# dotchen/LearningByCheating

Hardware: AMD Instinct MI355X
Metric: images/sec ImagePolicyModelSS phase-1 train @ bs256 (higher is better)
Workload: dtype bf16; 1 GPU; ImagePolicyModelSS(resnet34) phase-1 step vs BirdViewPolicyModelSS(resnet18) teacher [phase1_bs256_bf16], 160x384 RGB + 7x192x192 bird-view uint8 NHWC frames as the dataset stores them (2048-frame dataset per rank resident in HBM, a different batch every step), global batch 256 (256/GPU), bf16 MFMA operands and bf16 activation storage + f32 accumulate/master weights/gradients/BN/loss/Adam, local B; global_batch=256, parallelism=dp1

## Files before the change

learningbycheating_amd/csrc/conv_hdma.hip:

```cpp
#include "lbc_common.hpp"
#include "lbc_act.hpp"
#include "conv_lds_dma.hpp"


namespace {

struct HdmaCfg { int bm, bn, hrmax; };
const HdmaCfg kHdmaCfg[kLbcHdmaCfgs] = {{0, 0, 0}, {256, 128, 384}, {128, 256, 192}, {256, 64, 456}, {128, 64, 192}};
constexpr long long kHdmaSmallMinTiles = 48;

}

int lbc_conv_hdma_pick(const IgemmArgs& a, int mode)
{
    if (lbc_opt_on(kOptNoHdma) || lbc_opt_on(kOptNoGemm256)) return -1;
    if (a.nphase == 4) {
        if (!lbc_conv_hdmap_phased(a, mode) || lbc_opt(kOptGemm256Cfg) >= 0) return -1;
        const long long forcedp = lbc_opt(kOptHdmaCfg);
        if (forcedp >= 0 && forcedp != 4) return -1;
        const long long tiles = (long long)lbc_cdiv(a.M, 128) * (a.K / 64);
        const long long small_fill = lbc_opt(kOptGemm256MinTiles) > 0 ? lbc_opt(kOptGemm256MinTiles) : kHdmaSmallMinTiles;
        return tiles >= small_fill ? kLbcCfgHdma + 4 : -1;
    }
    if (!(a.w_bf16 && a.act_bf16) || a.ostep != 1 || a.nphase > 1 || a.oy0 || a.ox0) return -1;
    const bool c64 = a.C == 64 && a.K == 64;
    if (a.pre_scale && (mode != 0 || !c64 || lbc_opt_on(kOptNoC64pPre) || a.resid != nullptr)) return -1;
    if (a.KH != 3 || a.KW != 3 || a.P != 1 || a.S != 1 || a.C % 64 || (mode != 0 && mode != 1)) return -1;
    if (a.H != a.OH || a.W != a.OW || a.M != a.N * a.H * a.W || (long long)a.N * a.H * a.W * a.C >= (1ll << 31)) return -1;
    if ((long long)a.K * 9 * a.C >= (1ll << 31)) return -1;
    const long long fill = lbc_opt(kOptGemm256MinTiles) > 0 ? lbc_opt(kOptGemm256MinTiles) : 96;
    const long long forced = lbc_opt(kOptHdmaCfg);
    if (c64) {
        if (forced >= 0 && forced != 3) return -1;
        if (256 + 2 * a.W + 2 >= kHdmaCfg[3].hrmax || lbc_cdiv(a.M, 256) < fill) return -1;
        return kLbcCfgHdma + 3;
    }
    int best = -1;
    long long best_tiles = 0;
    double best_score = 0.0;
    for (int i = 1; i < 3; ++i) {
        const HdmaCfg& c = kHdmaCfg[i];
        if (a.K % c.bn) continue;
// ... 6 lines not shown
    }
    const long long below = lbc_opt(kOptHdmaSmallBelow) >= 0 ? lbc_opt(kOptHdmaSmallBelow) : 160;
    const bool prefer_small = best >= 0 && forced < 0 && best_tiles < below && a.K % 64 == 0 && lbc_opt(kOptGemm256MinTiles) <= 0 &&
                              lbc_conv_hdmap_eligible(a, mode, kLbcCfgHdma + 4);
    if (best >= 0 && !prefer_small) return kLbcCfgHdma + best;
    if ((forced < 0 || forced == 4) && a.K % 64 == 0 && lbc_conv_hdmap_eligible(a, mode, kLbcCfgHdma + 4)) {
        const long long tiles = (long long)lbc_cdiv(a.M, 128) * (a.K / 64);
        const long long small_fill = lbc_opt(kOptGemm256MinTiles) > 0 ? lbc_opt(kOptGemm256MinTiles) : kHdmaSmallMinTiles;
        if (tiles >= small_fill) return kLbcCfgHdma + 4;
    }
    return -1;
}

int lbc_conv_hdma_rows(const IgemmArgs& a, int cfg)
{
    if (cfg == kLbcCfgHdma + 3) return lbc_conv_c64p_rows(a);
    return lbc_cdiv(a.M, kHdmaCfg[cfg - kLbcCfgHdma].bm);
}

int lbc_conv_hdma_launch(const IgemmArgs& a, int mode, int cfg, hipStream_t s)
{
    LBC_REQUIRE(cfg > kLbcCfgHdma && cfg < kLbcCfgHdma + kLbcHdmaCfgs, "conv_hdma: bad cfg %d", cfg);
    const HdmaCfg c = kHdmaCfg[cfg - kLbcCfgHdma];
    LBC_REQUIRE(a.K % c.bn == 0 && a.C % 64 == 0 && c.bm + (a.nphase == 4 ? 1 : 2) * a.W + 2 < c.hrmax, "conv_hdma: shape not tileable");
    if (cfg == kLbcCfgHdma + 3) return lbc_conv_c64p_launch(a, mode, s);
    return lbc_conv_hdmap_launch(a, mode, cfg, s);
}
```

learningbycheating_amd/csrc/conv_hdmap.hip:

```cpp
#include "lbc_common.hpp"
#include "lbc_act.hpp"
#include "conv_hdmap.hpp"

int lbc_conv_hdmap_launch_256x128_320(const IgemmArgs& a, int mode, const void* zero, int ntiles, int tpw, unsigned grid, hipStream_t s);
int lbc_conv_hdmap_launch_256x128_384(const IgemmArgs& a, int mode, const void* zero, int ntiles, int tpw, unsigned grid, hipStream_t s);
int lbc_conv_hdmap_launch_128x256_192(const IgemmArgs& a, int mode, const void* zero, int ntiles, int tpw, unsigned grid, hipStream_t s);
int lbc_conv_hdmap_launch_128x64_192(const IgemmArgs& a, int mode, const void* zero, int ntiles, int tpw, unsigned grid, hipStream_t s, int nsplit, int kgroups);

namespace {

template <bool FUSED>
__global__ __launch_bounds__(256) void conv_split_epilogue_k(IgemmArgs a, const int nsplit)
{
    __shared__ float red[2][32][64];
    const int tid = threadIdx.x, rg = tid >> 3, seg = tid & 7;
    const int mt = blockIdx.x, n0 = blockIdx.y * 64, col = n0 + seg * 8;
    const size_t plane = (size_t)a.M * (size_t)a.K;
    __bf16* y = static_cast<__bf16*>(a.y);
    const __bf16* resid = static_cast<const __bf16*>(a.resid);
    const __bf16* by = static_cast<const __bf16*>(a.bnb_y);
    const __bf16* bmask = static_cast<const __bf16*>(a.bnb_mask);
    size_t o[4];
    bool live[4];
    f32x8 v[4];
#pragma unroll
    for (int q = 0; q < 4; ++q) {
        const int m = mt * 128 + rg + 32 * q;
        live[q] = m < a.M;
        o[q] = (size_t)(live[q] ? m : 0) * (size_t)a.K + (size_t)col;
        v[q] = ParamVec<8>::ld(a.split_ws + o[q]);
// ... 33 lines not shown
            u1 += t; u2 += t * t;
        }
        if (live[q]) *reinterpret_cast<bf16x8*>(y + o[q]) = ch;
    }
    if (a.stats) {
#pragma unroll
        for (int e = 0; e < 8; ++e) { red[0][rg][seg * 8 + e] = u1[e]; red[1][rg][seg * 8 + e] = u2[e]; }
        __syncthreads();
        if (tid < 128) {
            const int which = tid >> 6, c = tid & 63;
            float sum = 0.f;
#pragma unroll
            for (int r = 0; r < 32; ++r) sum += red[which][r][c];
            a.stats[(size_t)(a.stat_row0 + mt) * 2 * (size_t)a.K + (size_t)which * (size_t)a.K + (size_t)(n0 + c)] = sum;
        }
    }
}

}

int lbc_conv_hdmap_nsplit(const IgemmArgs& a, int mode, int cfg)
{
    (void)mode;
    if (cfg != kLbcCfgHdma + 4 || !a.split_ws || a.pre_scale || a.nphase == 4) return 1;
    const long long opt = lbc_opt(kOptHdmapSplit);
    if (opt == 0) return 1;
    const int nslab = a.C / 64;
    const long long tiles = (long long)lbc_cdiv(a.M, 128) * (a.K / 64), elems = (long long)a.M * a.K;
    auto fits = [&](long long n) { return n > 1 && nslab % n == 0 && elems * n <= a.split_ws_floats && elems * n < (1ll << 31); };
    if (opt > 1) return fits(opt) ? (int)opt : 1;
    if (tiles > 64 || nslab < 8) return 1;
    return fits(4) ? 4 : 1;
}

bool lbc_conv_hdmap_phased(const IgemmArgs& a, int mode)
{
    return mode == 1 && a.nphase == 4 && a.S == 2 && a.ostep == 2 && a.KH == 3 && a.KW == 3 && a.P == 1 && a.H == a.LH && a.W == a.LW &&
           a.OH == 2 * a.LH && a.OW == 2 * a.LW && a.M == a.N * a.LH * a.LW && !a.resid && !a.bnb_y && !a.pre_scale && a.w_bf16 && a.act_bf16 &&
           a.C % 64 == 0 && a.K % 64 == 0 && 128 + a.W + 2 <= 192 - 8 && (long long)a.N * a.OH * a.OW * a.K < (1ll << 31) &&
           (long long)a.N * a.H * a.W * a.C < (1ll << 31) && (long long)a.K * 9 * a.C < (1ll << 31) && !lbc_opt_on(kOptNoGldsPhased);
}

bool lbc_conv_hdmap_eligible(const IgemmArgs& a, int mode, int cfg)
{
    if (a.nphase == 4) return cfg == kLbcCfgHdma + 4 && lbc_conv_hdmap_phased(a, mode);
    if (mode != 0 && mode != 1) return false;
    if (a.pre_scale) return false;
    if (a.bnb_y && (mode != 1 || (a.resid != nullptr) != (a.bnb_mask != nullptr))) return false;
    if (cfg == kLbcCfgHdma + 1) return 256 + 2 * a.W + 2 <= 384 - 8;
    if (cfg == kLbcCfgHdma + 2 || cfg == kLbcCfgHdma + 4) return 128 + 2 * a.W + 2 <= 192 - 8;
    return false;
}

int lbc_conv_hdmap_launch(const IgemmArgs& a, int mode, int cfg, hipStream_t s)
{
    LBC_REQUIRE(lbc_conv_hdmap_eligible(a, mode, cfg), "conv_hdmap: launch not eligible");
    const int bm = cfg == kLbcCfgHdma + 1 ? 256 : 128, bn = cfg == kLbcCfgHdma + 1 ? 128 : (cfg == kLbcCfgHdma + 4 ? 64 : 256);
    LBC_REQUIRE(a.K % bn == 0 && a.C % 64 == 0, "conv_hdmap: shape not tileable");
    const void* zero = nullptr;
    int rc = lbc_zero_page(&zero);
    if (rc) return rc;
    const int ntiles = lbc_cdiv(a.M, bm) * (a.K / bn);
    const int cap = lbc_opt(kOptHdmaPersistWgs) > 0 ? (int)lbc_opt(kOptHdmaPersistWgs) : (cfg == kLbcCfgHdma + 4 ? 512 : 256);
    if (a.nphase == 4) {
        const int tpwp = lbc_cdiv(ntiles, cap);
        return lbc_conv_hdmap_launch_128x64_192(a, 2, zero, ntiles, tpwp, (unsigned)lbc_cdiv(ntiles, tpwp), s, 1, 1);
    }
    const int nsplit = lbc_conv_hdmap_nsplit(a, mode, cfg);
    if (nsplit > 1) {
        rc = lbc_conv_hdmap_launch_128x64_192(a, mode, zero, ntiles, 1, (unsigned)(ntiles * nsplit), s, nsplit, 1);
        if (rc) return rc;
        const dim3 eg((unsigned)lbc_cdiv(a.M, 128), (unsigned)(a.K / 64));
        if (a.bnb_y) hipLaunchKernelGGL(conv_split_epilogue_k<true>, eg, dim3(256), 0, s, a, nsplit);
        else hipLaunchKernelGGL(conv_split_epilogue_k<false>, eg, dim3(256), 0, s, a, nsplit);
        return lbc_check_launch("conv_split_epilogue");
    }
    if (cfg == kLbcCfgHdma + 4 && ntiles <= 256 && (a.C / 64) % 2 == 0 && (lbc_opt(kOptHdmapSplit) < 0 || lbc_opt(kOptHdmapSplit) == 1) && lbc_opt(kOptHdmaPersistWgs) <= 0)
        return lbc_conv_hdmap_launch_128x64_192(a, mode, zero, ntiles, 1, (unsigned)ntiles, s, 1, 2);
    const int tpw = lbc_cdiv(ntiles, cap);
    const unsigned grid = (unsigned)lbc_cdiv(ntiles, tpw);
    if (cfg == kLbcCfgHdma + 1) {
        if (256 + 2 * a.W + 2 <= 320 - 8) return lbc_conv_hdmap_launch_256x128_320(a, mode, zero, ntiles, tpw, grid, s);
        return lbc_conv_hdmap_launch_256x128_384(a, mode, zero, ntiles, tpw, grid, s);
    }
    if (cfg == kLbcCfgHdma + 4) return lbc_conv_hdmap_launch_128x64_192(a, mode, zero, ntiles, tpw, grid, s, 1, 1);
    return lbc_conv_hdmap_launch_128x256_192(a, mode, zero, ntiles, tpw, grid, s);
}
```

learningbycheating_amd/csrc/conv_hdmap.hpp:

```cpp
#pragma once
#include <type_traits>
#include "lbc_common.hpp"
#include "lbc_act.hpp"
#include "conv_lds_dma.hpp"

namespace {

#define LBC_SG(mask, n) __builtin_amdgcn_sched_group_barrier((mask), (n), 0)

__device__ __forceinline__ const char* uniform_ptr(const char* p)
{
    const unsigned long long v = (unsigned long long)(size_t)p;
    const unsigned lo = __builtin_amdgcn_readfirstlane((unsigned)v), hi = __builtin_amdgcn_readfirstlane((unsigned)(v >> 32));
    return reinterpret_cast<const char*>((size_t)(((unsigned long long)hi << 32) | lo));
}

template <int BM, int BN, int WM, int WN, int HRMAX, int SROWS>
constexpr int hdmap_lds_bytes() { return 2 * HRMAX * 128 + 3 * BN * 128 + WM * WN * SROWS * ((BN / WN) * 2 + 16) + WM * 2 * BN * 4; }
template <int BM, int BN, int WM, int WN, int HRMAX, int SROWS, int MODE, int EPI, int KG = 1>
__global__ __launch_bounds__(WM * WN * 64 * KG, (BM / WM == 128 && WM * WN == 4) ? 1 : 2) void conv_hdmap_k(IgemmArgs a, const void* zero_page, const int ntiles, const int tpw, const int nsplit)
{
    static_assert(KG == 1 || (KG == 2 && WM * WN == 4 && EPI != 3), "conv_hdmap: the in-workgroup K split doubles the four-wave shape");
    static_assert(MODE != 2 || (WM * WN == 4 && EPI == 0 && KG == 1), "conv_hdmap: the phased transposed form is a plain-epilogue form of the four-wave shape");
    constexpr int NPH = MODE == 2 ? 4 : 1;
    constexpr int WTM = BM / WM, WTN = BN / WN;
    constexpr int MT = WTM / 32, NT = WTN / 32;
    constexpr int NW = WM * WN;
    static_assert((NW == 8 || NW == 4) && (NT == 2 || NT == 1) && (MT == 2 || MT == 4), "conv_hdmap: wave tiling");
    static_assert(HRMAX % (8 * NW) == 0 && BN % (8 * NW) == 0 && (SROWS == 8 || SROWS == 16), "conv_hdmap: staging");
    constexpr int NB = 3;
    constexpr int KS = 4;
    constexpr int ABYTES = HRMAX * 128;
    constexpr int TILE_B = BN * 128;
    constexpr int BRING = 2 * ABYTES;
    constexpr int SROW_B = WTN * 2 + 16;
    constexpr int STG = BRING + NB * TILE_B;
    constexpr int RED = STG + NW * SROWS * SROW_B;
    constexpr int SMEM = RED + WM * 2 * BN * 4;
    static_assert(SMEM == hdmap_lds_bytes<BM, BN, WM, WN, HRMAX, SROWS>(), "conv_hdmap: LDS layout");
    constexpr int ZROW = (HRMAX - 1) * 128;
    static_assert(SMEM * KG <= 160 * 1024, "conv_hdmap: LDS");
    __shared__ __attribute__((aligned(16))) char smem_all[SMEM * KG];
    constexpr int HPW = HRMAX / (8 * NW);
    constexpr int NBW = BN / (8 * NW);
    constexpr int ATAPS = 7;
    constexpr int PPT = (HPW + ATAPS - 1) / ATAPS;
    static_assert(PPT >= 1 && PPT <= 2, "conv_hdmap: halo pieces per tap");
    constexpr int NSTEP = WTM / SROWS;
    constexpr int SEGS = WTN / 8;
    constexpr int CPL = SROWS * SEGS / 64;
    constexpr int RPP = 64 / SEGS;
    constexpr int NST = NSTEP * CPL;

    const int lane = threadIdx.x & 63;
    const int wave_all = __builtin_amdgcn_readfirstlane((int)threadIdx.x >> 6);
    const int grp = KG == 2 ? wave_all / NW : 0;
    const int wave = KG == 2 ? wave_all % NW : wave_all;
    const int tid = wave * 64 + lane;
    char* const smem = smem_all + grp * SMEM;
    const int wm = wave / WN, wn = wave % WN;
    const int l31 = lane & 31, kh = lane >> 5;
    const int W = a.W, H = a.H, C = a.C;
    const int ntn = a.K / BN;
    const int nslab = EPI == 3 ? C / 64 / nsplit : C / 64 / KG;

    int first, cnt, split = 0;
    {
        const int nwg = gridDim.x, b = blockIdx.x;
        const int xcd = b & 7, q = nwg >> 3, rr = nwg & 7;
        const int p = (xcd < rr ? xcd * (q + 1) : rr * (q + 1) + (xcd - rr) * q) + (b >> 3);
        if constexpr (EPI == 3) {
            first = p / nsplit;
            split = p - first * nsplit;
            cnt = first < ntiles ? 1 : 0;
        } else {
            first = p * tpw;
            cnt = ntiles - first < tpw ? ntiles - first : tpw;
        }
    }
    if (cnt <= 0) return;

    const __bf16* xin = static_cast<const __bf16*>(a.x) + (EPI == 3 ? split * nslab * 64 : (KG == 2 ? grp * nslab * 64 : 0));
    const __bf16* win = static_cast<const __bf16*>(a.w) + (EPI == 3 ? split * nslab * 64 : (KG == 2 ? grp * nslab * 64 : 0));
    const int prow = lane >> 3, pseg = lane & 7;

    const int HR = MODE == 2 ? BM + W + 2 : BM + 2 * W + 2;
    const int hshift = MODE == 2 ? 0 : W + 1;
    const int arow0 = wave * HPW * 8 + prow;
    const unsigned aswz[2] = {(unsigned)((pseg ^ ((arow0 >> 1) & 7)) * 16), (unsigned)((pseg ^ (((arow0 >> 1) + 4) & 7)) * 16)};
    const unsigned zoff = (unsigned)((lane & 7) * 16);
    const char* xbytes = reinterpret_cast<const char*>(xin);
    const char* zbytes = static_cast<const char*>(zero_page);
    auto issue_a = [&](const int m0x, const int slab, const int buf, const int j) {
        const bool pad = (wave * HPW + j) * 8 >= HR;
        int q = m0x - hshift + arow0 + 8 * j;
        q = q < 0 ? 0 : (q >= a.M ? a.M - 1 : q);
        const unsigned off = (unsigned)q * (unsigned)(2 * C) + aswz[j & 1];
        const char* sbase = uniform_ptr(pad ? zbytes : xbytes + (size_t)(slab * 128));
        lds_dma16(sbase + (pad ? zoff : off), smem + buf * ABYTES + (wave * HPW + j) * 1024);
    };
    unsigned voffb[NBW];
#pragma unroll
    for (int j = 0; j < NBW; ++j) {
        const int row = (wave * NBW + j) * 8 + prow;
        voffb[j] = (unsigned)row * (unsigned)(18 * C) + (unsigned)((pseg ^ ((row >> 1) & 7)) * 16);
    }
    const char* wbytes = reinterpret_cast<const char*>(win);
    auto issue_b = [&](const int n0x, const int slab, const int tap, const int slot, const int j0, const int j1) {
        char* base = smem + BRING + slot * TILE_B;
        const char* wsrc = uniform_ptr(wbytes + ((size_t)n0x * (size_t)(18 * C) + (size_t)(2 * (tap * C + slab * 64))));
#pragma unroll
        for (int j = 0; j < NBW; ++j)
            if (j >= j0 && j < j1) lds_dma16(wsrc + voffb[j], base + (wave * NBW + j) * 1024);
    };
    const int baddr = (BRING + (wn * WTN + l31) * 128) | ((kh ^ ((l31 >> 1) & 7)) << 4);
    int rowc[MT];
#pragma unroll
    for (int i = 0; i < MT; ++i) rowc[i] = hshift + wm * WTM + i * 32 + l31;
    auto tap_mask = [&](const int m0x, int (&mask)[MT]) {
#pragma unroll
        for (int i = 0; i < MT; ++i) {
            const int m = m0x + wm * WTM + i * 32 + l31;
            int bits = 0;
            if (m < a.M) {
                const int x = m % W;
                const int y = (m / W) % H;
#pragma unroll
                for (int t = 0; t < 9; ++t) {
                    const int r = t / 3, s = t - 3 * r;
                    const int dy = MODE == 0 ? r - 1 : (MODE == 2 ? (r == 0 ? 1 : 0) : 1 - r);
                    const int dx = MODE == 0 ? s - 1 : (MODE == 2 ? (s == 0 ? 1 : 0) : 1 - s);
                    if ((unsigned)(y + dy) < (unsigned)H && (unsigned)(x + dx) < (unsigned)W) bits |= 1 << t;
                }
            }
            mask[i] = bits;
        }
    };
    int amask[MT], amaskn[MT];

    f32x16 acc[NPH][MT][NT];
    auto zero_acc = [&]() {
#pragma unroll
        for (int p = 0; p < NPH; ++p)
#pragma unroll
            for (int i = 0; i < MT; ++i)
#pragma unroll
                for (int j = 0; j < NT; ++j)
#pragma unroll
                    for (int r = 0; r < 16; ++r) acc[p][i][j][r] = 0.f;
    };
    zero_acc();

    int aaddr[MT];
    auto tap_addr = [&](const int tap, const int buf, const int (&mask)[MT]) {
        const int r = tap / 3, s = tap - 3 * r;
        const int off = MODE == 0 ? (r - 1) * W + (s - 1) : (MODE == 2 ? (r == 0 ? W : 0) + (s == 0 ? 1 : 0) : (1 - r) * W + (1 - s));
        const int abuf = buf * ABYTES;
#pragma unroll
        for (int i = 0; i < MT; ++i) {
            const int hr = rowc[i] + off;
            const int val = (hr << 7) | ((kh ^ ((hr >> 1) & 7)) << 4), zval = ZROW | (kh << 4);
            const int m = -((mask[i] >> tap) & 1);
            aaddr[i] = abuf + (((val ^ zval) & m) ^ zval);
        }
    };

    bf16x8 fa[2][MT], fb[2][NT];
    constexpr bool ASMRD = NB * TILE_B + (NT - 1) * 4096 < 65536;
    const unsigned lds0 = (unsigned)(size_t)(__attribute__((address_space(3))) char*)smem_all + (unsigned)(grp * SMEM);
#ifdef LBC_HIP_EMULATED_FOR_TESTS
#define LBC_RD1(DST, ADDR, OFF) DST = *reinterpret_cast<const bf16x8*>(smem + (ADDR) + (OFF))
#define LBC_USE(SET) do { } while (0)
#else
#define LBC_RD1(DST, ADDR, OFF)                                                                                                  \
    do {                                                                                                                         \
        if constexpr (ASMRD) asm volatile("ds_read_b128 %0, %1 offset:%2" : "=v"(DST) : "v"(lds0 + (unsigned)(ADDR)), "n"(OFF)); \
        else DST = *reinterpret_cast<const bf16x8*>(smem + (ADDR) + (OFF));                                                      \
    } while (0)
#define LBC_USE(SET)                                                                                                             \
// ... 7 lines not shown
#define LBC_WAIT_OLDER_READS() do { if constexpr (ASMRD) __builtin_amdgcn_s_waitcnt(waitcnt_imm(63, MT + NT)); } while (0)
#define LBC_RD(SLOT, G, SET)                                                                                                     \
    do {                                                                                                                         \
        _Pragma("unroll") for (int i = 0; i < MT; ++i) LBC_RD1(fa[SET][i], aaddr[i] ^ (32 * (G)), 0);                            \
        if constexpr (NT == 2) { LBC_RD1(fb[SET][0], baddr ^ (32 * (G)), (SLOT) * TILE_B); LBC_RD1(fb[SET][NT - 1], baddr ^ (32 * (G)), (SLOT) * TILE_B + 4096); } \
        else LBC_RD1(fb[SET][0], baddr ^ (32 * (G)), (SLOT) * TILE_B);                                                           \
    } while (0)
#define LBC_MM(SET, PHX)                                                                                                         \
    do {                                                                                                                         \
        _Pragma("unroll") for (int i = 0; i < MT; ++i)                                                                           \
            _Pragma("unroll") for (int j = 0; j < NT; ++j)                                                                       \
                acc[PHX][i][j] = __builtin_amdgcn_mfma_f32_32x32x16_bf16(fa[SET][i], fb[SET][j], acc[PHX][i][j], 0, 0, 0);       \
    } while (0)

    auto wait_vm = [&](const int n) {
        switch (n) {
#define LBC_WV(N) case N: LBC_WAIT_VM(N); break;
            LBC_WV(1) LBC_WV(2) LBC_WV(3) LBC_WV(4) LBC_WV(5) LBC_WV(6) LBC_WV(7) LBC_WV(8) LBC_WV(9) LBC_WV(10) LBC_WV(11) LBC_WV(12)
            LBC_WV(13) LBC_WV(14) LBC_WV(15) LBC_WV(16) LBC_WV(17) LBC_WV(18) LBC_WV(19) LBC_WV(20) LBC_WV(21) LBC_WV(22) LBC_WV(23) LBC_WV(24)
#undef LBC_WV
            default: LBC_WAIT_VM(0); break;
        }
    };
    static_assert(NBW + 2 * PPT + NPH * NST <= 24, "conv_hdmap: counted waits");

    int tile = first;
    int mtile = tile / ntn, n0 = (tile - mtile * ntn) * BN, m0 = mtile * BM;
    int sg = 0;
    tap_mask(m0, amask);

#pragma unroll
    for (int j = 0; j < HPW; ++j) issue_a(m0, 0, 0, j);
    issue_b(n0, 0, 0, 0, 0, NBW);
    issue_b(n0, 0, 1, 1, 0, NBW);
    LBC_WAIT_VM(NBW);
    __builtin_amdgcn_s_barrier();
    tap_addr(0, 0, amask);
    LBC_RD(0, 0, 0);
    bool stores_pending = false;
    for (int it = 0; it < cnt; ++it) {
        const bool more = it + 1 < cnt;
        const int tilen = tile + 1;
        const int mtilen = tilen / ntn, n0n = (tilen - mtilen * ntn) * BN, m0n = mtilen * BM;
        if (more) tap_mask(m0n, amaskn);

        auto slab_body = [&](const int c, auto last_tag) {
            constexpr bool LAST = decltype(last_tag)::value;
            const bool follows = !LAST || more;
#pragma unroll
            for (int i = 0; i < MT; ++i) asm volatile("" : "+v"(rowc[i]), "+v"(amask[i]));
            const int buf = sg & 1;
#pragma unroll
            for (int t = 0; t < 9; ++t) {
                const int slot = t % 3, nslot = (t + 1) % 3, islot = (t + 2) % 3;
                const int tph = MODE == 2 ? (t / 3 == 1 ? 0 : 2) + (t % 3 == 1 ? 0 : 1) : 0;
                const bool has_next = t < 8 || follows;
                const bool w2 = t + 2 < 9 || follows;
                const int np_here = (t * PPT < HPW ? (HPW - t * PPT < PPT ? HPW - t * PPT : PPT) : 0);
                const int np_prev = t >= 1 ? ((t - 1) * PPT < HPW ? (HPW - (t - 1) * PPT < PPT ? HPW - (t - 1) * PPT : PPT) : 0) : 0;
                const bool hp = np_here > 0 && follows;
                auto issue_w = [&](const int j0, const int j1) {
                    if (!w2) return;
                    const int tt = t + 2 < 9 ? t + 2 : t - 7;
                    const int cc = t + 2 < 9 ? c : (LAST ? 0 : c + 1);
                    const int nn = (t + 2 < 9 || !LAST) ? n0 : n0n;
                    issue_b(nn, cc, tt, islot, j0, j1);
                };
                auto issue_h = [&]() {
                    if (!hp) return;
#pragma unroll
                    for (int q = 0; q < PPT; ++q)
                        if (t * PPT + q < HPW) {
                            if (!LAST) issue_a(m0, c + 1, buf ^ 1, t * PPT + q);
                            else issue_a(m0n, 0, buf ^ 1, t * PPT + q);
                        }
                };
#pragma unroll
                for (int g = 0; g + 1 < KS; ++g) {
                    LBC_RD(slot, g + 1, (g + 1) & 1);
                    if (g == KS - 2 && has_next) {
                        if (t < 8) tap_addr(t + 1, buf, amask);
                        else if (!LAST) tap_addr(0, buf ^ 1, amask);
                        else tap_addr(0, buf ^ 1, amaskn);
                    }
                    if (g == 0) issue_w(0, NBW / 2);
                    else if (g == 1) issue_w(NBW / 2, NBW);
                    else issue_h();
                    LBC_WAIT_OLDER_READS();
                    LBC_USE(g & 1);
                    LBC_MM(g & 1, tph);
                    LBC_SG(0x100, MT + NT);
#pragma unroll
                    for (int q = 0; q < MT * NT; ++q) { LBC_SG(0x008, 1); LBC_SG(0x036, 5); }
                    __builtin_amdgcn_sched_barrier(0);
                }
                {
                    int n = 0;
                    if (w2) {
                        n = NBW + (follows ? np_prev + np_here : 0);
                        if (c == 0 && t == 0 && stores_pending) n += NPH * NST;
                    }
                    wait_vm(n);
                }
                LBC_WAIT_LGKM0();
                __builtin_amdgcn_s_barrier();
                __builtin_amdgcn_sched_barrier(0);
                if (has_next) LBC_RD(nslot, 0, 0);
                LBC_USE((KS - 1) & 1);
                LBC_MM((KS - 1) & 1, tph);
                LBC_SG(0x100, MT + NT);
#pragma unroll
                for (int q = 0; q < MT * NT; ++q) { LBC_SG(0x008, 1); LBC_SG(0x036, 6); }
                __builtin_amdgcn_sched_barrier(0);
            }
            ++sg;
        };
        for (int c = 0; c + 1 < nslab; ++c) slab_body(c, std::false_type{});
        slab_body(nslab - 1, std::true_type{});

        if constexpr (KG == 2) {
            static_assert(NW * MT * NT * 16 * 64 * 4 <= 2 * ABYTES, "conv_hdmap: accumulator hand-over buffer");
            float* xch = reinterpret_cast<float*>(smem_all + SMEM) + (size_t)wave * (MT * NT * 16 * 64) + lane;
// ... 176 lines not shown
                            red[(wm * 2 + 1) * BN + wn * WTN + nj * 32 + l31] = s2[nj];
                        }
                    }
                }
                LBC_WAIT_LGKM0();
                __builtin_amdgcn_s_barrier();
                if (epi_on && tid < BN) {
                    float u1 = 0.f, u2 = 0.f;
#pragma unroll
                    for (int w2 = 0; w2 < WM; ++w2) { u1 += red[(w2 * 2 + 0) * BN + tid]; u2 += red[(w2 * 2 + 1) * BN + tid]; }
                    float* dst = a.stats + (size_t)(a.stat_row0 + ph * (ntiles / ntn) + mtile) * 2 * (size_t)a.K;
                    dst[n0 + tid] = u1;
                    dst[a.K + n0 + tid] = u2;
                }
                if constexpr (NPH > 1) { LBC_WAIT_LGKM0(); __builtin_amdgcn_s_barrier(); }
            }
            }
        }
        zero_acc();
        stores_pending = true;
        tile = tilen; mtile = mtilen; n0 = n0n; m0 = m0n;
#pragma unroll
        for (int i = 0; i < MT; ++i) amask[i] = amaskn[i];
    }
#undef LBC_RD
#undef LBC_RD1
#undef LBC_USE
#undef LBC_WAIT_OLDER_READS
#undef LBC_MM
}
#undef LBC_SG

template <int BM, int BN, int WM, int WN, int HRMAX, int SROWS>
int conv_hdmap_launch_shape(const IgemmArgs& a, int mode, const void* zero, int ntiles, int tpw, dim3 grid, hipStream_t s, int nsplit = 1, int kgroups = 1)
{
    if (nsplit > 1) {
        if constexpr (BM == 128 && BN == 64) {
            LBC_REQUIRE(a.split_ws && tpw == 1 && grid.x == (unsigned)(ntiles * nsplit) && (a.C / 64) % nsplit == 0, "conv_hdmap: bad split-K launch");
            if (mode == 0) hipLaunchKernelGGL((conv_hdmap_k<BM, BN, WM, WN, HRMAX, SROWS, 0, 3>), grid, dim3(WM * WN * 64), 0, s, a, zero, ntiles, tpw, nsplit);
            else hipLaunchKernelGGL((conv_hdmap_k<BM, BN, WM, WN, HRMAX, SROWS, 1, 3>), grid, dim3(WM * WN * 64), 0, s, a, zero, ntiles, tpw, nsplit);
            return lbc_check_launch("conv_hdmap(split)");
        } else {
            LBC_REQUIRE(false, "conv_hdmap: split-K exists for the 128 x 64 shape only");
        }
    }
    const int epi = a.bnb_y ? (a.bnb_mask ? 4 : 2) : (a.resid ? 1 : 0);
// ... 41 lines not shown
```

learningbycheating_amd/csrc/conv_igemm.hip:

```cpp
#include "lbc_common.hpp"
#include "lbc_act.hpp"
#include <type_traits>
#include <stdlib.h>

namespace {

template <int BM, int BN, bool WMAJOR, int MODE, bool BF16, typename AT, typename WT, int PF, int BKV = 0, bool X3 = false>
__global__ __launch_bounds__(256, PF == 2 ? 2 : 1) void conv_igemm_k(IgemmArgs a)
{
    static_assert(!BF16 || WMAJOR, "the bf16 path needs depth-contiguous weights");
    static_assert(!X3 || (BF16 && !Act<AT>::kBf16 && !Act<WT>::kBf16), "the split path reads f32 tensors and f32 weights");
    static_assert(!Act<AT>::kBf16 || BF16, "bf16 activations need the bf16 MFMA path");
    static_assert(!Act<WT>::kBf16 || BF16, "bf16 weights need the bf16 MFMA path");
    constexpr bool ABF = Act<AT>::kBf16;
    constexpr bool WBF = Act<WT>::kBf16;
    using breg_t = typename std::conditional<WBF, bf16x8, f32x4>::type;
    constexpr int BEL = WBF ? 8 : 4;
    using areg_t = typename std::conditional<ABF, bf16x8, f32x4>::type;
    using lds_t = typename std::conditional<BF16, __bf16, float>::type;
    constexpr int BK = BKV ? BKV : (BF16 ? 64 : 32);
    constexpr int LDK = (X3 ? 2 * BK : BK) + (BF16 ? 8 : 4);
    constexpr int LO = X3 ? BK : 0;
    constexpr int SEGS = BK / BEL;
    constexpr int RPP = 256 / SEGS;
// ... 498 lines not shown
    LBC_REQUIRE(!a.bf16 || wmajor, "igemm: the bf16 path needs depth-contiguous weights (transpose first)");
    LBC_REQUIRE(!a.act_bf16 || a.bf16, "igemm: bf16 activations need bf16 = 1");
    LBC_REQUIRE(!a.w_bf16 || a.act_bf16, "igemm: bf16 weight copies are used with bf16 activations only");
    LBC_REQUIRE(!a.x3 || (a.bf16 && !a.act_bf16), "igemm: split-bf16 operands need bf16 = 1 on f32 tensors");
    LBC_REQUIRE(cfg >= kLbcCfgGlds || a.K % kCfgBN[cfg] == 0, "igemm: output channels %d not a multiple of the tile", a.K);
    LBC_REQUIRE(a.KH * a.KW <= 16, "igemm: too many taps");
    LBC_REQUIRE(a.S == 1 || a.S == 2, "igemm: stride %d unsupported", a.S);
    LBC_REQUIRE(a.M > 0, "igemm: empty launch");
    LBC_REQUIRE((long long)a.N * a.H * a.W * a.C < (1ll << 31) && (long long)a.N * a.OH * a.OW * a.K < (1ll << 31),
                "igemm: tensor exceeds 2^31 elements");
    LBC_REQUIRE(a.nphase == 0 || a.nphase == 1 || (a.nphase == 4 && mode == 1 && a.S == 2 && a.ostep == 2), "igemm: bad nphase %d", a.nphase);
    double taps = 0;
    for (int t = 0; t < a.KH * a.KW; ++t) {
        const int r = t / a.KW, q = t - r * a.KW;
        if (a.nphase == 4) { taps += 0.25; continue; }
        if (mode == 1 && a.S == 2 && ((((a.oy0 + a.P - r) & 1) != 0) || (((a.ox0 + a.P - q) & 1) != 0))) continue;
        taps += 1;
    }
    const double nph = a.nphase == 4 ? 4.0 : 1.0;
    const double in_elems = (double)a.N * a.H * a.W * a.C * ((mode == 1 && a.S == 2) ? nph / 4.0 : 1.0);
    const bool halo = cfg < kLbcCfgGlds && wmajor && lbc_conv3x3_halo_eligible(a, mode);
    const bool ksplit = cfg >= kLbcCfgHdma && lbc_conv_hdmap_nsplit(a, mode, cfg) > 1;
    const char* pname = ksplit ? (mode == 0 ? "conv_hdma_gather_split" : "conv_hdma_transposed_split")
                        : cfg >= kLbcCfgHdma ? (mode == 0 ? "conv_hdma_gather" : "conv_hdma_transposed")
                        : cfg >= kLbcCfgGlds ? (mode == 0 ? "conv_glds_gather" : "conv_glds_transposed")
                        : halo ? (mode == 0 ? "conv_halo_gather" : "conv_halo_transposed")
                        : a.x3 ? (mode == 0 ? "conv_igemm_x3_gather" : "conv_igemm_x3_transposed")
                               : (mode == 0 ? "conv_igemm_gather" : "conv_igemm_transposed");
    LbcProfScope prof(pname, 2.0 * a.M * nph * a.K * (double)a.C * taps,
                      (a.act_bf16 ? 2.0 : 4.0) * (in_elems + nph * (double)a.M * a.K * (1 + (a.resid ? 1 : 0) + (a.bnb_y ? 1 : 0) + (a.bnb_mask ? 1 : 0))) +
                          (a.w_bf16 ? 2.0 : 4.0) * taps * nph * a.C * a.K, s);
    if (lbc_prof_on() && (a.bnb_y || a.bnb_mask))
        lbc_prof_note("side_tensors_of_fused_reduce", (a.act_bf16 ? 2.0 : 4.0) * nph * (double)a.M * a.K * ((a.bnb_y ? 1 : 0) + (a.bnb_mask ? 1 : 0)));
    if (cfg >= kLbcCfgHdma) {
        LBC_REQUIRE(wmajor && lbc_conv_hdma_pick(a, mode) >= 0, "igemm: launch not eligible for the halo-staged LDS-DMA kernel");
        return lbc_conv_hdma_launch(a, mode, cfg, s);
    }
    if (cfg >= kLbcCfgGlds) {
        LBC_REQUIRE(wmajor && lbc_conv_glds_pick(a, mode) >= 0, "igemm: launch not eligible for the 8-wave LDS-DMA kernel");
        return lbc_conv_glds_launch(a, mode, cfg, s);
    }
    if (wmajor && lbc_conv3x3_halo_eligible(a, mode)) return lbc_conv3x3_halo_launch(a, mode, s);
    switch (cfg) {
        case 0: return launch_cfg<128, 64>(a, wmajor, mode, s);
        case 1: return launch_cfg<128, 128>(a, wmajor, mode, s);
        default: return launch_cfg<64, 64>(a, wmajor, mode, s);
    }
// ... 2 lines not shown
```

learningbycheating_amd/csrc/lbc_common.hpp:

```cpp
#pragma once
#include <hip/hip_runtime.h>
#include <stddef.h>
#include <stdint.h>

typedef float f32x4 __attribute__((ext_vector_type(4)));
typedef float f32x16 __attribute__((ext_vector_type(16)));

#define LBC_OK 0
#define LBC_EINVAL (-1)
#define LBC_ELAUNCH (-2)
#define LBC_ESTATE (-3)

void lbc_set_error(const char* fmt, ...);
int lbc_check_launch(const char* what);

#define LBC_REQUIRE(cond, ...)                 \
    do {                                       \
        if (!(cond)) {                         \
            lbc_set_error(__VA_ARGS__);        \
            return LBC_EINVAL;                 \
        }                                      \
    } while (0)

static inline int lbc_cdiv(long long a, long long b) { return (int)((a + b - 1) / b); }

enum LbcOpt {
    kOptForceCfg = 0,
    kOptHaloBlocks,
    kOptHeadNoMfma,
    kOptNoSideStream,
    kOptNoGemm256,
    kOptGemm256MinTiles,
    kOptGemm256Cfg,
    kOptNoBnBwdFuse,
    kOptNoHdma,
    kOptHdmaCfg,
    kOptNoGldsPhased,
    kOptHdmaPersistWgs,
    kOptWgradTr2MinWgs,
    kOptNoC64pPre,
    kOptNoBnFold,
    kOptC64pBm,
    kOptHdmapSplit,
    kOptHdmaSmallBelow,
    kOptCount
};
long long lbc_opt(LbcOpt o);
static inline bool lbc_opt_on(LbcOpt o) { return lbc_opt(o) == 1; }

bool lbc_prof_on();
void lbc_prof_begin(const char* name, double flops, double bytes, hipStream_t s);
void lbc_prof_end(hipStream_t s);
void lbc_prof_note(const char* name, double bytes);
struct LbcProfScope {
    hipStream_t s; bool on;
    LbcProfScope(const char* name, double flops, double bytes, hipStream_t st) : s(st), on(lbc_prof_on()) {
        if (on) lbc_prof_begin(name, flops, bytes, s);
    }
    ~LbcProfScope() { if (on) lbc_prof_end(s); }
};

struct IgemmArgs {
    const void* x;
    const void* w;
    void* y;
    const float* post_scale;
// ... 38 lines not shown
};
static inline int lbc_weight_prep_tiles(int A, int T, int B) { return lbc_cdiv(A, 64) * lbc_cdiv(B, 64) * T; }
struct WeightPrepArgs {
    static const int kMax = 48;
    WeightPrepItem item[kMax];
    int count;
    int tiles;
};
int lbc_weight_prep(const WeightPrepArgs& a, hipStream_t s);

int lbc_igemm_rows(const IgemmArgs& a, int cfg);
int lbc_igemm_pick(long long M, int K);
int lbc_igemm_pick_for(const IgemmArgs& a, int mode);
constexpr int kLbcCfgGlds = 3;
constexpr int kLbcGldsCfgs = 7;
constexpr int kLbcCfgHdma = kLbcCfgGlds + kLbcGldsCfgs;
constexpr int kLbcHdmaCfgs = 5;
int lbc_conv_hdma_pick(const IgemmArgs& a, int mode);
int lbc_conv_hdma_rows(const IgemmArgs& a, int cfg);
int lbc_conv_hdma_launch(const IgemmArgs& a, int mode, int cfg, hipStream_t s);
int lbc_conv_c64p_launch(const IgemmArgs& a, int mode, hipStream_t s);
int lbc_conv_c64p_rows(const IgemmArgs& a);
bool lbc_conv_hdmap_phased(const IgemmArgs& a, int mode);
bool lbc_conv_hdmap_eligible(const IgemmArgs& a, int mode, int cfg);
int lbc_conv_hdmap_launch(const IgemmArgs& a, int mode, int cfg, hipStream_t s);
int lbc_conv_hdmap_nsplit(const IgemmArgs& a, int mode, int cfg);
int lbc_conv_glds_pick(const IgemmArgs& a, int mode);
int lbc_conv_glds_rows(const IgemmArgs& a, int cfg);
int lbc_conv_glds_launch(const IgemmArgs& a, int mode, int cfg, hipStream_t s);
int lbc_zero_page(const void** p);
int lbc_igemm_launch(const IgemmArgs& a, int wmajor, int mode, int cfg, hipStream_t s);
int lbc_weight_transpose(const float* w, float* wt, int A, int T, int B, hipStream_t s);
bool lbc_conv3x3_halo_eligible(const IgemmArgs& a, int mode);
int lbc_conv3x3_halo_launch(const IgemmArgs& a, int mode, hipStream_t s);

struct WgradArgs {
    const void* p;
    const void* q;
    float* partial;
    const float* p_scale;
    const float* p_shift;
    const float* q_scale;
    const float* q_shift;
    int q_relu;
    int N, OH, OW, CP;
    int H, W, CQ;
// ... 29 lines not shown
```

learningbycheating_amd/csrc/lbc_util.cpp:

```cpp
#include "lbc_common.hpp"
#include <stdarg.h>
#include <stdio.h>

static thread_local char g_err[512] = "";

void lbc_set_error(const char* fmt, ...)
{
    va_list ap;
    va_start(ap, fmt);
    vsnprintf(g_err, sizeof(g_err), fmt, ap);
    va_end(ap);
}

int lbc_check_launch(const char* what)
{
    hipError_t e = hipGetLastError();
    if (e != hipSuccess) {
        lbc_set_error("%s: launch failed: %s", what, hipGetErrorString(e));
        return LBC_ELAUNCH;
    }
    return LBC_OK;
}

extern "C" const char* lbc_last_error(void) { return g_err; }

#include <stdlib.h>
#include <mutex>
extern "C" char** environ;
#include <string.h>
namespace {
const char* const kOptNames[kOptCount] = {
    "LBC_FORCE_CFG", "LBC_HALO_BLOCKS", "LBC_HEAD_NO_MFMA", "LBC_NO_SIDE_STREAM", "LBC_NO_GEMM256", "LBC_GEMM256_MIN_TILES", "LBC_GEMM256_CFG",
    "LBC_NO_BN_BWD_FUSE", "LBC_NO_HDMA", "LBC_HDMA_CFG", "LBC_NO_GLDS_PHASED", "LBC_HDMA_PERSIST_WGS", "LBC_WGRAD_TR2_MIN_WGS", "LBC_NO_C64P_PRE",
    "LBC_NO_BN_FOLD", "LBC_C64P_BM", "LBC_HDMAP_SPLIT", "LBC_HDMA_SMALL_BELOW"};
struct OptTable {
    long long v[kOptCount];
    OptTable()
    {
        for (int i = 0; i < kOptCount; ++i) {
            const char* e = getenv(kOptNames[i]);
            v[i] = (e && *e) ? atoll(e) : -1;
        }
        for (char** ep = environ; ep && *ep; ++ep) {
            if (strncmp(*ep, "LBC_", 4)) continue;
            const char* eq = strchr(*ep, '=');
            const size_t n = eq ? (size_t)(eq - *ep) : strlen(*ep);
            bool known = (n == 17 && !strncmp(*ep, "LBC_PROF_LAUNCHES", n)) || (n == 15 && !strncmp(*ep, "LBC_PIN_STAGING", n)) || !strncmp(*ep, "LBC_ARCH", 8) || !strncmp(*ep, "LBC_BUILD_", 10) || !strncmp(*ep, "LBC_TEST_", 9) || !strncmp(*ep, "LBC_EMU_", 8);
            for (int i = 0; i < kOptCount && !known; ++i) known = strlen(kOptNames[i]) == n && !strncmp(*ep, kOptNames[i], n);
            if (!known) fprintf(stderr, "liblbc_hip: environment variable %.*s is not an option of this library (ignored); see include/lbc_hip.h, lbc_config_set\n", (int)n, *ep);
        }
    }
};
OptTable& opts() { static OptTable t; return t; }
}
long long lbc_opt(LbcOpt o) { return opts().v[o]; }
extern "C" int lbc_config_set(const char* name, long long value)
{
// ... 91 lines not shown
```

Measured before the change: 17360 images/sec.

## Add stride-2 3x3 forward conv path to LDS-DMA halo kernel

Adds a MODE 3 variant of the persistent LDS-DMA implicit-GEMM conv kernel for stride-2 3x3 forward convolutions. Input pixels are gathered per stride phase into LDS halo buffers, and the taps are reordered so each phase's halo load is reused across the taps that read it. Eligible ResNet downsampling convs are routed to this kernel instead of the generic igemm path, with a new option to disable it. It adds a more complex wait/issue schedule and new index arithmetic, which carries correctness and pipelining risk.

Result: no change. 17460 images/sec, median of 6 (+0.6%).

```diff
diff --git a/learningbycheating_amd/csrc/conv_hdma.hip b/learningbycheating_amd/csrc/conv_hdma.hip
--- a/learningbycheating_amd/csrc/conv_hdma.hip
+++ b/learningbycheating_amd/csrc/conv_hdma.hip
@@ -18,6 +18,14 @@
         if (!lbc_conv_hdmap_phased(a, mode) || lbc_opt(kOptGemm256Cfg) >= 0) return -1;
         const long long forcedp = lbc_opt(kOptHdmaCfg);
         if (forcedp >= 0 && forcedp != 4) return -1;
+        const long long tiles = (long long)lbc_cdiv(a.M, 128) * (a.K / 64);
+        const long long small_fill = lbc_opt(kOptGemm256MinTiles) > 0 ? lbc_opt(kOptGemm256MinTiles) : kHdmaSmallMinTiles;
+        return tiles >= small_fill ? kLbcCfgHdma + 4 : -1;
+    }
+    if (a.S == 2 && lbc_conv_hdmap_s2gather(a, mode)) {
+        if (lbc_opt(kOptGemm256Cfg) >= 0) return -1;
+        const long long forceds = lbc_opt(kOptHdmaCfg);
+        if (forceds >= 0 && forceds != 4) return -1;
         const long long tiles = (long long)lbc_cdiv(a.M, 128) * (a.K / 64);
         const long long small_fill = lbc_opt(kOptGemm256MinTiles) > 0 ? lbc_opt(kOptGemm256MinTiles) : kHdmaSmallMinTiles;
         return tiles >= small_fill ? kLbcCfgHdma + 4 : -1;
@@ -70,7 +78,7 @@
 {
     LBC_REQUIRE(cfg > kLbcCfgHdma && cfg < kLbcCfgHdma + kLbcHdmaCfgs, "conv_hdma: bad cfg %d", cfg);
     const HdmaCfg c = kHdmaCfg[cfg - kLbcCfgHdma];
-    LBC_REQUIRE(a.K % c.bn == 0 && a.C % 64 == 0 && c.bm + (a.nphase == 4 ? 1 : 2) * a.W + 2 < c.hrmax, "conv_hdma: shape not tileable");
+    LBC_REQUIRE(a.K % c.bn == 0 && a.C % 64 == 0 && c.bm + (a.S == 2 && a.nphase != 4 ? a.OW : (a.nphase == 4 ? 1 : 2) * a.W) + 2 < c.hrmax, "conv_hdma: shape not tileable");
     if (cfg == kLbcCfgHdma + 3) return lbc_conv_c64p_launch(a, mode, s);
     return lbc_conv_hdmap_launch(a, mode, cfg, s);
 }
diff --git a/learningbycheating_amd/csrc/conv_hdmap.hip b/learningbycheating_amd/csrc/conv_hdmap.hip
--- a/learningbycheating_amd/csrc/conv_hdmap.hip
+++ b/learningbycheating_amd/csrc/conv_hdmap.hip
@@ -6,6 +6,7 @@
 int lbc_conv_hdmap_launch_256x128_384(const IgemmArgs& a, int mode, const void* zero, int ntiles, int tpw, unsigned grid, hipStream_t s);
 int lbc_conv_hdmap_launch_128x256_192(const IgemmArgs& a, int mode, const void* zero, int ntiles, int tpw, unsigned grid, hipStream_t s);
 int lbc_conv_hdmap_launch_128x64_192(const IgemmArgs& a, int mode, const void* zero, int ntiles, int tpw, unsigned grid, hipStream_t s, int nsplit, int kgroups);
+int lbc_conv_hdmap_launch_s2_128x64_192(const IgemmArgs& a, const void* zero, int ntiles, int tpw, unsigned grid, hipStream_t s);
 
 namespace {
 
@@ -85,7 +86,7 @@
 int lbc_conv_hdmap_nsplit(const IgemmArgs& a, int mode, int cfg)
 {
     (void)mode;
-    if (cfg != kLbcCfgHdma + 4 || !a.split_ws || a.pre_scale || a.nphase == 4) return 1;
+    if (cfg != kLbcCfgHdma + 4 || !a.split_ws || a.pre_scale || a.nphase == 4 || a.S != 1) return 1;
     const long long opt = lbc_opt(kOptHdmapSplit);
     if (opt == 0) return 1;
     const int nslab = a.C / 64;
@@ -104,9 +105,18 @@
            (long long)a.N * a.H * a.W * a.C < (1ll << 31) && (long long)a.K * 9 * a.C < (1ll << 31) && !lbc_opt_on(kOptNoGldsPhased);
 }
 
+bool lbc_conv_hdmap_s2gather(const IgemmArgs& a, int mode)
+{
+    return mode == 0 && a.S == 2 && a.KH == 3 && a.KW == 3 && a.P == 1 && a.ostep == 1 && a.nphase <= 1 && !a.oy0 && !a.ox0 && a.H == 2 * a.OH &&
+           a.W == 2 * a.OW && a.M == a.N * a.OH * a.OW && !a.resid && !a.bnb_y && !a.pre_scale && a.w_bf16 && a.act_bf16 && a.C % 64 == 0 &&
+           a.K % 64 == 0 && 128 + a.OW + 2 <= 192 - 8 && (long long)a.N * a.OH * a.OW * a.K < (1ll << 31) &&
+           (long long)a.N * a.H * a.W * a.C < (1ll << 31) && (long long)a.K * 9 * a.C < (1ll << 31) && !lbc_opt_on(kOptNoHdmaS2);
+}
+
 bool lbc_conv_hdmap_eligible(const IgemmArgs& a, int mode, int cfg)
 {
     if (a.nphase == 4) return cfg == kLbcCfgHdma + 4 && lbc_conv_hdmap_phased(a, mode);
+    if (a.S != 1) return cfg == kLbcCfgHdma + 4 && lbc_conv_hdmap_s2gather(a, mode);
     if (mode != 0 && mode != 1) return false;
     if (a.pre_scale) return false;
     if (a.bnb_y && (mode != 1 || (a.resid != nullptr) != (a.bnb_mask != nullptr))) return false;
@@ -129,6 +139,10 @@
         const int tpwp = lbc_cdiv(ntiles, cap);
         return lbc_conv_hdmap_launch_128x64_192(a, 2, zero, ntiles, tpwp, (unsigned)lbc_cdiv(ntiles, tpwp), s, 1, 1);
     }
+    if (a.S != 1) {
+        const int tpws = lbc_cdiv(ntiles, cap);
+        return lbc_conv_hdmap_launch_s2_128x64_192(a, zero, ntiles, tpws, (unsigned)lbc_cdiv(ntiles, tpws), s);
+    }
     const int nsplit = lbc_conv_hdmap_nsplit(a, mode, cfg);
     if (nsplit > 1) {
         rc = lbc_conv_hdmap_launch_128x64_192(a, mode, zero, ntiles, 1, (unsigned)(ntiles * nsplit), s, nsplit, 1);
diff --git a/learningbycheating_amd/csrc/conv_hdmap.hpp b/learningbycheating_amd/csrc/conv_hdmap.hpp
--- a/learningbycheating_amd/csrc/conv_hdmap.hpp
+++ b/learningbycheating_amd/csrc/conv_hdmap.hpp
@@ -15,6 +15,9 @@
     return reinterpret_cast<const char*>((size_t)(((unsigned long long)hi << 32) | lo));
 }
 
+constexpr int hdmap_s2_tap(int t) { constexpr int seq[9] = {0, 2, 6, 8, 3, 5, 1, 7, 4}; return seq[t]; }
+constexpr int hdmap_s2_phase(int t) { return t < 4 ? 3 : (t < 6 ? 1 : (t < 8 ? 2 : 0)); }
+constexpr int hdmap_s2_buf(int t) { return t < 4 ? 0 : (t < 6 ? 1 : (t < 8 ? 0 : 1)); }
 template <int BM, int BN, int WM, int WN, int HRMAX, int SROWS>
 constexpr int hdmap_lds_bytes() { return 2 * HRMAX * 128 + 3 * BN * 128 + WM * WN * SROWS * ((BN / WN) * 2 + 16) + WM * 2 * BN * 4; }
 template <int BM, int BN, int WM, int WN, int HRMAX, int SROWS, int MODE, int EPI, int KG = 1>
@@ -22,6 +25,7 @@
 {
     static_assert(KG == 1 || (KG == 2 && WM * WN == 4 && EPI != 3), "conv_hdmap: the in-workgroup K split doubles the four-wave shape");
     static_assert(MODE != 2 || (WM * WN == 4 && EPI == 0 && KG == 1), "conv_hdmap: the phased transposed form is a plain-epilogue form of the four-wave shape");
+    static_assert(MODE != 3 || (WM * WN == 4 && EPI == 0 && KG == 1), "conv_hdmap: the stride-2 gather form is a plain-epilogue form of the four-wave shape");
     constexpr int NPH = MODE == 2 ? 4 : 1;
     constexpr int WTM = BM / WM, WTN = BN / WN;
     constexpr int MT = WTM / 32, NT = WTN / 32;
@@ -46,6 +50,7 @@
     constexpr int ATAPS = 7;
     constexpr int PPT = (HPW + ATAPS - 1) / ATAPS;
     static_assert(PPT >= 1 && PPT <= 2, "conv_hdmap: halo pieces per tap");
+    constexpr int PA3 = (HPW + 2) / 3;
     constexpr int NSTEP = WTM / SROWS;
     constexpr int SEGS = WTN / 8;
     constexpr int CPL = SROWS * SEGS / 64;
@@ -60,7 +65,7 @@
     char* const smem = smem_all + grp * SMEM;
     const int wm = wave / WN, wn = wave % WN;
     const int l31 = lane & 31, kh = lane >> 5;
-    const int W = a.W, H = a.H, C = a.C;
+    const int W = MODE == 3 ? a.OW : a.W, H = MODE == 3 ? a.OH : a.H, C = a.C;
     const int ntn = a.K / BN;
     const int nslab = EPI == 3 ? C / 64 / nsplit : C / 64 / KG;
 
@@ -84,7 +89,7 @@
     const __bf16* win = static_cast<const __bf16*>(a.w) + (EPI == 3 ? split * nslab * 64 : (KG == 2 ? grp * nslab * 64 : 0));
     const int prow = lane >> 3, pseg = lane & 7;
 
-    const int HR = MODE == 2 ? BM + W + 2 : BM + 2 * W + 2;
+    const int HR = MODE == 2 || MODE == 3 ? BM + W + 2 : BM + 2 * W + 2;
     const int hshift = MODE == 2 ? 0 : W + 1;
     const int arow0 = wave * HPW * 8 + prow;
     const unsigned aswz[2] = {(unsigned)((pseg ^ ((arow0 >> 1) & 7)) * 16), (unsigned)((pseg ^ (((arow0 >> 1) + 4) & 7)) * 16)};
@@ -99,6 +104,25 @@
         const char* sbase = uniform_ptr(pad ? zbytes : xbytes + (size_t)(slab * 128));
         lds_dma16(sbase + (pad ? zoff : off), smem + buf * ABYTES + (wave * HPW + j) * 1024);
     };
+    unsigned apix[MODE == 3 ? HPW : 1], apixn[MODE == 3 ? HPW : 1];
+    auto halo_pix = [&](const int m0x, unsigned (&pix)[MODE == 3 ? HPW : 1]) {
+        if constexpr (MODE == 3) {
+#pragma unroll
+            for (int j = 0; j < HPW; ++j) {
+                int q = m0x - hshift + arow0 + 8 * j;
+                q = q < 0 ? 0 : (q >= a.M ? a.M - 1 : q);
+                pix[j] = (unsigned)(4 * q - 2 * (q % W));
+            }
+        }
+    };
+    auto issue_a3 = [&](const unsigned (&pix)[MODE == 3 ? HPW : 1], const int slab, const int ph, const int buf, const int j) {
+        if constexpr (MODE == 3) {
+            const bool pad = (wave * HPW + j) * 8 >= HR;
+            const unsigned off = pix[j] * (unsigned)(2 * C) + aswz[j & 1];
+            const char* sbase = uniform_ptr(pad ? zbytes : xbytes + ((size_t)(slab * 128) + (size_t)((ph >> 1) * 2 * W + (ph & 1)) * (size_t)(2 * C)));
+            lds_dma16(sbase + (pad ? zoff : off), smem + buf * ABYTES + (wave * HPW + j) * 1024);
+        }
+    };
     unsigned voffb[NBW];
 #pragma unroll
     for (int j = 0; j < NBW; ++j) {
@@ -128,8 +152,8 @@
 #pragma unroll
                 for (int t = 0; t < 9; ++t) {
                     const int r = t / 3, s = t - 3 * r;
-                    const int dy = MODE == 0 ? r - 1 : (MODE == 2 ? (r == 0 ? 1 : 0) : 1 - r);
-                    const int dx = MODE == 0 ? s - 1 : (MODE == 2 ? (s == 0 ? 1 : 0) : 1 - s);
+                    const int dy = MODE == 0 ? r - 1 : (MODE == 2 ? (r == 0 ? 1 : 0) : (MODE == 3 ? (r == 0 ? -1 : 0) : 1 - r));
+                    const int dx = MODE == 0 ? s - 1 : (MODE == 2 ? (s == 0 ? 1 : 0) : (MODE == 3 ? (s == 0 ? -1 : 0) : 1 - s));
                     if ((unsigned)(y + dy) < (unsigned)H && (unsigned)(x + dx) < (unsigned)W) bits |= 1 << t;
                 }
             }
@@ -154,7 +178,7 @@
     int aaddr[MT];
     auto tap_addr = [&](const int tap, const int buf, const int (&mask)[MT]) {
         const int r = tap / 3, s = tap - 3 * r;
-        const int off = MODE == 0 ? (r - 1) * W + (s - 1) : (MODE == 2 ? (r == 0 ? W : 0) + (s == 0 ? 1 : 0) : (1 - r) * W + (1 - s));
+        const int off = MODE == 0 ? (r - 1) * W + (s - 1) : (MODE == 2 ? (r == 0 ? W : 0) + (s == 0 ? 1 : 0) : (MODE == 3 ? -((r == 0 ? W : 0) + (s == 0 ? 1 : 0)) : (1 - r) * W + (1 - s)));
         const int abuf = buf * ABYTES;
 #pragma unroll
         for (int i = 0; i < MT; ++i) {
@@ -208,49 +232,69 @@
             default: LBC_WAIT_VM(0); break;
         }
     };
-    static_assert(NBW + 2 * PPT + NPH * NST <= 24, "conv_hdmap: counted waits");
+    static_assert(NBW + 2 * PPT + NPH * NST <= 24 && (MODE != 3 || NBW + HPW + NST <= 24), "conv_hdmap: counted waits");
+    auto tap_of = [](const int t) { return MODE == 3 ? hdmap_s2_tap(t) : t; };
 
     int tile = first;
     int mtile = tile / ntn, n0 = (tile - mtile * ntn) * BN, m0 = mtile * BM;
     int sg = 0;
     tap_mask(m0, amask);
-
-#pragma unroll
-    for (int j = 0; j < HPW; ++j) issue_a(m0, 0, 0, j);
-    issue_b(n0, 0, 0, 0, 0, NBW);
-    issue_b(n0, 0, 1, 1, 0, NBW);
+    halo_pix(m0, apix);
+
+#pragma unroll
+    for (int j = 0; j < HPW; ++j) {
+        if constexpr (MODE == 3) issue_a3(apix, 0, hdmap_s2_phase(0), 0, j);
+        else issue_a(m0, 0, 0, j);
+    }
+    issue_b(n0, 0, tap_of(0), 0, 0, NBW);
+    issue_b(n0, 0, tap_of(1), 1, 0, NBW);
     LBC_WAIT_VM(NBW);
     __builtin_amdgcn_s_barrier();
-    tap_addr(0, 0, amask);
+    tap_addr(tap_of(0), 0, amask);
     LBC_RD(0, 0, 0);
     bool stores_pending = false;
     for (int it = 0; it < cnt; ++it) {
         const bool more = it + 1 < cnt;
         const int tilen = tile + 1;
         const int mtilen = tilen / ntn, n0n = (tilen - mtilen * ntn) * BN, m0n = mtilen * BM;
-        if (more) tap_mask(m0n, amaskn);
+        if (more) { tap_mask(m0n, amaskn); halo_pix(m0n, apixn); }
 
         auto slab_body = [&](const int c, auto last_tag) {
             constexpr bool LAST = decltype(last_tag)::value;
             const bool follows = !LAST || more;
 #pragma unroll
             for (int i = 0; i < MT; ++i) asm volatile("" : "+v"(rowc[i]), "+v"(amask[i]));
-            const int buf = sg & 1;
+            const int buf0 = sg & 1;
 #pragma unroll
             for (int t = 0; t < 9; ++t) {
                 const int slot = t % 3, nslot = (t + 1) % 3, islot = (t + 2) % 3;
+                const int buf = MODE == 3 ? hdmap_s2_buf(t) : buf0;
                 const int tph = MODE == 2 ? (t / 3 == 1 ? 0 : 2) + (t % 3 == 1 ? 0 : 1) : 0;
                 const bool has_next = t < 8 || follows;
                 const bool w2 = t + 2 < 9 || follows;
-                const int np_here = (t * PPT < HPW ? (HPW - t * PPT < PPT ? HPW - t * PPT : PPT) : 0);
-                const int np_prev = t >= 1 ? ((t - 1) * PPT < HPW ? (HPW - (t - 1) * PPT < PPT ? HPW - (t - 1) * PPT : PPT) : 0) : 0;
-                const bool hp = np_here > 0 && follows;
+                const int p3_lo = t < 3 ? (t * PA3 < HPW ? t * PA3 : HPW) : 0;
+                const int p3_hi = t < 3 ? ((t + 1) * PA3 < HPW ? (t + 1) * PA3 : HPW) : ((t == 4 || t == 6 || t == 8) ? HPW : 0);
+                const bool forced3 = MODE == 3 && t == 8;
+                const int np_here = MODE == 3 ? (forced3 ? 0 : p3_hi - p3_lo)
+                                              : (t * PPT < HPW ? (HPW - t * PPT < PPT ? HPW - t * PPT : PPT) : 0);
+                const int np_prev = MODE == 3 ? 0 : (t >= 1 ? ((t - 1) * PPT < HPW ? (HPW - (t - 1) * PPT < PPT ? HPW - (t - 1) * PPT : PPT) : 0) : 0);
+                const bool hp = (MODE == 3 ? p3_hi > p3_lo && (t < 8 || follows) : np_here > 0 && follows);
                 auto issue_w = [&](const int j0, const int j1) {
                     if (!w2) return;
                     const int tt = t + 2 < 9 ? t + 2 : t - 7;
                     const int cc = t + 2 < 9 ? c : (LAST ? 0 : c + 1);
                     const int nn = (t + 2 < 9 || !LAST) ? n0 : n0n;
-                    issue_b(nn, cc, tt, islot, j0, j1);
+                    issue_b(nn, cc, tap_of(tt), islot, j0, j1);
+                };
+                auto issue_h3 = [&](const int j0, const int j1) {
+                    if (!hp) return;
+#pragma unroll
+                    for (int j = 0; j < HPW; ++j)
+                        if (j >= j0 && j < j1) {
+                            if (t < 8) issue_a3(apix, c, hdmap_s2_phase(t < 4 ? 4 : t + 2), buf ^ 1, j);
+                            else if (!LAST) issue_a3(apix, c + 1, hdmap_s2_phase(0), buf ^ 1, j);
+                            else issue_a3(apixn, 0, hdmap_s2_phase(0), buf ^ 1, j);
+                        }
                 };
                 auto issue_h = [&]() {
                     if (!hp) return;
@@ -265,13 +309,20 @@
                 for (int g = 0; g + 1 < KS; ++g) {
                     LBC_RD(slot, g + 1, (g + 1) & 1);
                     if (g == KS - 2 && has_next) {
-                        if (t < 8) tap_addr(t + 1, buf, amask);
-                        else if (!LAST) tap_addr(0, buf ^ 1, amask);
-                        else tap_addr(0, buf ^ 1, amaskn);
-                    }
-                    if (g == 0) issue_w(0, NBW / 2);
-                    else if (g == 1) issue_w(NBW / 2, NBW);
-                    else issue_h();
+                        if (t < 8) tap_addr(tap_of(t + 1), MODE == 3 ? hdmap_s2_buf(t + 1) : buf, amask);
+                        else if (!LAST) tap_addr(tap_of(0), buf ^ 1, amask);
+                        else tap_addr(tap_of(0), buf ^ 1, amaskn);
+                    }
+                    if constexpr (MODE == 3) {
+                        const int mid = (p3_lo + p3_hi + 1) / 2;
+                        if (g == 0) issue_h3(p3_lo, mid);
+                        else if (g == 1) { issue_h3(mid, p3_hi); issue_w(0, NBW / 2); }
+                        else issue_w(NBW / 2, NBW);
+                    } else {
+                        if (g == 0) issue_w(0, NBW / 2);
+                        else if (g == 1) issue_w(NBW / 2, NBW);
+                        else issue_h();
+                    }
                     LBC_WAIT_OLDER_READS();
                     LBC_USE(g & 1);
                     LBC_MM(g & 1, tph);
@@ -283,7 +334,7 @@
                 {
                     int n = 0;
                     if (w2) {
-                        n = NBW + (follows ? np_prev + np_here : 0);
+                        n = NBW + (MODE == 3 ? (hp ? np_here : 0) : (follows ? np_prev + np_here : 0));
                         if (c == 0 && t == 0 && stores_pending) n += NPH * NST;
                     }
                     wait_vm(n);
@@ -506,6 +557,10 @@
         tile = tilen; mtile = mtilen; n0 = n0n; m0 = m0n;
 #pragma unroll
         for (int i = 0; i < MT; ++i) amask[i] = amaskn[i];
+        if constexpr (MODE == 3) {
+#pragma unroll
+            for (int j = 0; j < HPW; ++j) apix[j] = apixn[j];
+        }
     }
 #undef LBC_RD
 #undef LBC_RD1
diff --git a/learningbycheating_amd/csrc/conv_hdmap_128x64_192_s2.hip b/learningbycheating_amd/csrc/conv_hdmap_128x64_192_s2.hip
--- /dev/null
+++ b/learningbycheating_amd/csrc/conv_hdmap_128x64_192_s2.hip
@@ -0,0 +1,9 @@
+#include "conv_hdmap.hpp"
+
+int lbc_conv_hdmap_launch_s2_128x64_192(const IgemmArgs& a, const void* zero, int ntiles, int tpw, unsigned grid, hipStream_t s)
+{
+    LBC_REQUIRE(!a.resid && !a.bnb_y && !a.pre_scale && a.S == 2 && a.H == 2 * a.OH && a.W == 2 * a.OW && 128 + a.OW + 2 <= 192 - 8,
+                "conv_hdmap: the stride-2 gather form has the plain epilogue and even input extents only");
+    hipLaunchKernelGGL((conv_hdmap_k<128, 64, 2, 2, 192, 16, 3, 0>), dim3(grid), dim3(256), 0, s, a, zero, ntiles, tpw, 1);
+    return lbc_check_launch("conv_hdmap(s2)");
+}
diff --git a/learningbycheating_amd/csrc/conv_igemm.hip b/learningbycheating_amd/csrc/conv_igemm.hip
--- a/learningbycheating_amd/csrc/conv_igemm.hip
+++ b/learningbycheating_amd/csrc/conv_igemm.hip
@@ -544,7 +544,7 @@
     const bool halo = cfg < kLbcCfgGlds && wmajor && lbc_conv3x3_halo_eligible(a, mode);
     const bool ksplit = cfg >= kLbcCfgHdma && lbc_conv_hdmap_nsplit(a, mode, cfg) > 1;
     const char* pname = ksplit ? (mode == 0 ? "conv_hdma_gather_split" : "conv_hdma_transposed_split")
-                        : cfg >= kLbcCfgHdma ? (mode == 0 ? "conv_hdma_gather" : "conv_hdma_transposed")
+                        : cfg >= kLbcCfgHdma ? (mode == 0 ? (a.S == 2 ? "conv_hdma_gather_s2" : "conv_hdma_gather") : "conv_hdma_transposed")
                         : cfg >= kLbcCfgGlds ? (mode == 0 ? "conv_glds_gather" : "conv_glds_transposed")
                         : halo ? (mode == 0 ? "conv_halo_gather" : "conv_halo_transposed")
                         : a.x3 ? (mode == 0 ? "conv_igemm_x3_gather" : "conv_igemm_x3_transposed")
diff --git a/learningbycheating_amd/csrc/lbc_common.hpp b/learningbycheating_amd/csrc/lbc_common.hpp
--- a/learningbycheating_amd/csrc/lbc_common.hpp
+++ b/learningbycheating_amd/csrc/lbc_common.hpp
@@ -42,6 +42,7 @@
     kOptNoBnFold,
     kOptC64pBm,
     kOptHdmapSplit,
+    kOptNoHdmaS2,
     kOptHdmaSmallBelow,
     kOptCount
 };
@@ -126,6 +127,7 @@
 int lbc_conv_c64p_launch(const IgemmArgs& a, int mode, hipStream_t s);
 int lbc_conv_c64p_rows(const IgemmArgs& a);
 bool lbc_conv_hdmap_phased(const IgemmArgs& a, int mode);
+bool lbc_conv_hdmap_s2gather(const IgemmArgs& a, int mode);
 bool lbc_conv_hdmap_eligible(const IgemmArgs& a, int mode, int cfg);
 int lbc_conv_hdmap_launch(const IgemmArgs& a, int mode, int cfg, hipStream_t s);
 int lbc_conv_hdmap_nsplit(const IgemmArgs& a, int mode, int cfg);
diff --git a/learningbycheating_amd/csrc/lbc_util.cpp b/learningbycheating_amd/csrc/lbc_util.cpp
--- a/learningbycheating_amd/csrc/lbc_util.cpp
+++ b/learningbycheating_amd/csrc/lbc_util.cpp
@@ -32,7 +32,7 @@
 const char* const kOptNames[kOptCount] = {
     "LBC_FORCE_CFG", "LBC_HALO_BLOCKS", "LBC_HEAD_NO_MFMA", "LBC_NO_SIDE_STREAM", "LBC_NO_GEMM256", "LBC_GEMM256_MIN_TILES", "LBC_GEMM256_CFG",
     "LBC_NO_BN_BWD_FUSE", "LBC_NO_HDMA", "LBC_HDMA_CFG", "LBC_NO_GLDS_PHASED", "LBC_HDMA_PERSIST_WGS", "LBC_WGRAD_TR2_MIN_WGS", "LBC_NO_C64P_PRE",
-    "LBC_NO_BN_FOLD", "LBC_C64P_BM", "LBC_HDMAP_SPLIT", "LBC_HDMA_SMALL_BELOW"};
+    "LBC_NO_BN_FOLD", "LBC_C64P_BM", "LBC_HDMAP_SPLIT", "LBC_NO_HDMA_S2", "LBC_HDMA_SMALL_BELOW"};
 struct OptTable {
     long long v[kOptCount];
     OptTable()
```
